# mcmilk/7-Zip-zstd

Hardware: AMD Instinct MI355X
Metric: compress MB/s + ratio-vs-ref, enwik9 zstd-L3 & Silesia flzma2-L5 (value = the zstd-L3 enwik9 leg; flzma2_l5_silesia = the other leg) (higher is better)
Workload: dtype u8; 1 GPU; zstd level 3, enwik9 stand-in (text-zipf, 1000000000 B), 128 KiB blocks in independent 8 MiB match-finder frames; bytes_total=1000000000

## Files before the change

### 7-zip-zstd_amd/csrc/gc_api.hip

```cpp
#include "gpucodec.h"
#include "gc_common.h"
#include "gc_lzma2.h"
#include "gc_brotli.h"
#include "gc_mf.h"
#include "gc_zstd_dec.h"
#include "gc_brotli_dec.h"
#include "gc_lzma2_dec_work.h"
#ifdef HIPEMU
#include "hip_runtime_stub.h"
#else
#include <hip/hip_runtime.h>
#define GC_LAUNCH(kernel, grid, block, stream, ...) hipLaunchKernelGGL(kernel, dim3(grid), dim3(block), 0, stream, __VA_ARGS__)
#endif
#include <stdio.h>
#include <stdlib.h>
#include <string.h>
#include <new>
#include "gc_host_stream.h"
#ifdef GC_TEST_HOOKS
#include <vector>
#include <unistd.h>
#endif

struct GcFramePlan { uint64_t off; uint32_t size; uint32_t compressed; };
// ... 399 lines not shown
#define GC_MF_ENT_BUDGET ((size_t)24u << 30)
static uint32_t mf_auto_parts(size_t n, uint32_t frameArg)
{
    if (MF_F(frameArg) <= 1u) return 1u;
    const size_t perGroup = (size_t)MF_FPG(frameArg) * MF_F(frameArg) * GC_ZSTD_BLOCK_MAX * sizeof(GcMfEntry);
    const size_t nGroups = (gc_num_blocks(n) + MF_C(frameArg) - 1u) / MF_C(frameArg);
    size_t perPart = GC_MF_ENT_BUDGET / perGroup; if (perPart < 1u) perPart = 1u;
    size_t parts = (nGroups + perPart - 1u) / perPart;
    return (uint32_t)(parts < 1u ? 1u : (parts > GC_MAX_PARTS ? GC_MAX_PARTS : parts));
}
static int ensure_finder_workspace(gc_ctx* c, const GcLzPlan& plan, size_t n, uint32_t frameBlocks, size_t maxPartBytes = 0 )
{
    if (MF_F(frameBlocks) <= 1u) return GC_OK;
    const GcMfGeom g = gc_mf_geom(n, frameBlocks, plan.mfFast != 0u);
    const GcMfGeom gp = gc_mf_geom(maxPartBytes && maxPartBytes < n ? maxPartBytes : n, frameBlocks, plan.mfFast != 0u);
    const size_t needCnt = gp.cntWords * sizeof(uint32_t), needEnt = (size_t)gp.nFrames * gp.frameBytes * sizeof(GcMfEntry);
    const size_t needRec = (size_t)g.nBlocks * GC_ZSTD_BLOCK_MAX * sizeof(uint32_t);
    const size_t needPrice = (size_t)g.nBlocks * GC_PRICE_WORDS * sizeof(uint16_t);
    const size_t needTileWord = ((size_t)g.nTiles + 64u) * sizeof(uint32_t);
    if (needTileWord > c->mfTileWordCap || needCnt > c->mfCntCap || needEnt > c->mfEntCap || needEnt > c->mfEnt2Cap || needRec > c->mfRecCap || ((plan.searchDepth || plan.shortPass) && (needRec > c->mfRec2Cap || needRec / 32u + 64u > c->mfChangedCap)) ||
        (plan.priceParse && (needRec / 2u > c->mfRec3Cap || needRec > c->mfDpCap || needPrice > c->mfPriceCap || (size_t)g.nBlocks * 128u > c->mfWinCostCap || (size_t)g.nBlocks * GC_DPS_WORDS * 4u > c->mfDpStatCap || needRec / 4u > c->mfLitPriceCap))) {
        HIPCHK(c, hipStreamSynchronize(c->stream));
        int rc;
        if ((rc = mf_grow(c, (void**)&c->mfTileWord, &c->mfTileWordCap, needTileWord, "tile counts")) != GC_OK) return rc;
        if ((rc = mf_grow(c, (void**)&c->mfCnt, &c->mfCntCap, needCnt, "offsets")) != GC_OK) return rc;
        if ((rc = mf_grow(c, (void**)&c->mfEnt, &c->mfEntCap, needEnt, "entries")) != GC_OK) return rc;
        if ((rc = mf_grow(c, (void**)&c->mfEnt2, &c->mfEnt2Cap, needEnt, "linked entries")) != GC_OK) return rc;
        if ((rc = mf_grow(c, (void**)&c->mfRec, &c->mfRecCap, needRec, "records")) != GC_OK) return rc;
        if ((plan.searchDepth || plan.shortPass) && (rc = mf_grow(c, (void**)&c->mfRec2, &c->mfRec2Cap, needRec, "deepened records")) != GC_OK) return rc;
        if ((plan.searchDepth || plan.shortPass) && (rc = mf_grow(c, (void**)&c->mfChanged, &c->mfChangedCap, needRec / 32u + 64u, "changed-record bitmap")) != GC_OK) return rc;
        if (plan.priceParse) {
            if ((rc = mf_grow(c, (void**)&c->mfRec3, &c->mfRec3Cap, needRec / 2u, "short candidates")) != GC_OK) return rc;
            if ((rc = mf_grow(c, (void**)&c->mfDp, &c->mfDpCap, needRec, "price-parse records")) != GC_OK) return rc;
            if ((rc = mf_grow(c, (void**)&c->mfPrice, &c->mfPriceCap, needPrice, "price tables")) != GC_OK) return rc;
            if ((rc = mf_grow(c, (void**)&c->mfWinCost, &c->mfWinCostCap, (size_t)g.nBlocks * 128u, "window costs")) != GC_OK) return rc;
            if ((rc = mf_grow(c, (void**)&c->mfDpStat, &c->mfDpStatCap, (size_t)g.nBlocks * GC_DPS_WORDS * 4u, "path symbol counts")) != GC_OK) return rc;
            if ((rc = mf_grow(c, (void**)&c->mfLitPrice, &c->mfLitPriceCap, needRec / 4u, "literal prices")) != GC_OK) return rc;
        }
    }
    return GC_OK;
}

static int launch_finder_part(gc_ctx* c, const GcLzPlan& plan, hipStream_t st, uint32_t part, const uint8_t* src, size_t n, uint32_t frameArg , uint32_t blk0, unsigned long long* prof)
{
    const uint32_t frameBlocks = frameArg;
    const uint32_t groupBlocks = MF_C(frameArg);
    const uint32_t nBlocks = gc_num_blocks(n);
    GcSeqRaw* seqRaw = c->seqRaw + (size_t)blk0 * GC_MAX_SEQ_PER_BLOCK;
    uint8_t* lit = c->lit + (size_t)blk0 * GC_ZSTD_BLOCK_MAX;
    GcBlockMeta* meta = c->meta + blk0;
    if (MF_F(frameArg) <= 1u) {
        GC_LAUNCH(gc_zstd_lz_kernel, nBlocks, 1024, st, src, (uint64_t)n, seqRaw, lit, meta, prof);
        return GC_OK;
    }
    const GcMfGeom g = gc_mf_geom(n, frameBlocks, plan.mfFast != 0u);
    const uint32_t frame0 = (blk0 / groupBlocks) * MF_FPG(frameArg);
    uint32_t* cnt = c->mfCnt;
    GcMfEntry* ent = c->mfEnt;
    GcMfEntry* ent2 = c->mfEnt2;
    uint32_t* rec = c->mfRec + (size_t)blk0 * GC_ZSTD_BLOCK_MAX;
    const uint32_t perT = gc_xcd_per(g.nTiles), perB = gc_xcd_per(nBlocks);
    const bool fast = plan.mfFast != 0u;
    const uint32_t nParts = 1u << g.partLog;
#define MFSEL(k) (fast ? k##_p8 : k)
    uint32_t linkLaunch = 0;
    const uint32_t linkWpc = 6u;
    const uint32_t nLists = g.nFrames * nParts, linkGrid = nLists * GC_MF_LINK_SEGS < c->nCU * linkWpc ? nLists * GC_MF_LINK_SEGS : c->nCU * linkWpc;
    HIPCHK(c, hipMemsetAsync(c->mfTicket + part * 16u, 0, 16u * sizeof(uint32_t), st));
#define MF_LINK(cnt_, ent_, ent2_) do { uint32_t* ticket_ = c->mfTicket + part * 16u + linkLaunch++; \
        GC_LAUNCH(MFSEL(gc_mf_link_kernel), linkGrid, 64, st, (const uint32_t*)(cnt_), (const GcMfEntry*)(ent_), ent2_, g.tilesPerFrame, g.frameBytes, nLists, ticket_); } while (0)
    hipEvent_t* ev = c->evMf[part];
    HIPCHK(c, hipEventRecord(ev[0], st));
    const bool shortBeside = plan.priceParse && st == c->stream;
    if (shortBeside) {
        HIPCHK(c, hipEventRecord(c->evShort[part], st)); HIPCHK(c, hipStreamWaitEvent(c->stream2, c->evShort[part], 0));
        const uint32_t nChunkWg = (uint32_t)(((n + 2047u) / 2048u + 3u) / 4u), perC = gc_xcd_per(nChunkWg);
        GC_LAUNCH(gc_mf_short_kernel, perC * GC_XCDS, 256, c->stream2, src, (uint64_t)n, groupBlocks, (uint32_t)((n + 2047u) / 2048u), perC, c->mfRec3 + (size_t)blk0 * GC_ZSTD_BLOCK_MAX);
        HIPCHK(c, hipEventRecord(c->evShort[part], c->stream2));
    }
    GC_LAUNCH(MFSEL(gc_mf_count_kernel), perT * GC_XCDS, nParts, st, src, (uint64_t)n, frameBlocks, g.nTiles, perT, cnt);
    HIPCHK(c, hipEventRecord(ev[1], st));
    GC_LAUNCH(MFSEL(gc_mf_scan_kernel), g.nFrames, 1024, st, cnt, g.tilesPerFrame);
    HIPCHK(c, hipEventRecord(ev[2], st));
    GC_LAUNCH(MFSEL(gc_mf_scatter_kernel), perT * GC_XCDS, nParts, st, src, (uint64_t)n, frameBlocks, g.nTiles, perT, (const uint32_t*)cnt, ent);
    HIPCHK(c, hipEventRecord(ev[3], st));
    MF_LINK(cnt, ent, ent2);
    HIPCHK(c, hipEventRecord(ev[4], st));
    const bool fused = !plan.farPass && !plan.farPass2 && !plan.searchDepth && !plan.priceParse && !plan.shortPass && MF_C(frameArg) == MF_F(frameArg);
    if (fused) {
        {
            const uint32_t tpb = GC_ZSTD_BLOCK_MAX >> g.tileLog;
            const uint32_t perV = ((gc_xcd_per(g.nTiles) + tpb - 1u) / tpb) * tpb;
            uint32_t* tw = c->mfTileWord + (size_t)frame0 * g.tilesPerFrame;
            HIPCHK(c, hipMemsetAsync(tw, 0, (size_t)g.nTiles * sizeof(uint32_t), st));
            GC_LAUNCH(MFSEL(gc_mf_vparse_tile_kernel), perV * GC_XCDS, g.verifyT, st, src, (uint64_t)n, frameBlocks, g.nTiles, perV, plan.lazyDepth, (const uint32_t*)cnt,
                      (const GcMfEntry*)ent2, seqRaw, lit, meta, c->mfTicket + part * 16u + 8u, tw, prof);
        }
        for (int i = 10; i <= 12; i++) HIPCHK(c, hipEventRecord(ev[i], st));
        HIPCHK(c, hipEventRecord(ev[5], st));
        HIPCHK(c, hipEventRecord(ev[6], st));
        (void)prof;
        return GC_OK;
    }
    GC_LAUNCH(MFSEL(gc_mf_verify_kernel), perT * GC_XCDS, g.verifyT, st, src, (uint64_t)n, frameBlocks, g.nTiles, perT, (const uint32_t*)cnt,
                   (const GcMfEntry*)ent2, rec);
    HIPCHK(c, hipEventRecord(ev[10], st));
    if (plan.farPass) {
        GC_LAUNCH(MFSEL(gc_mf_count_far_kernel), perT * GC_XCDS, nParts, st, src, (uint64_t)n, frameBlocks, g.nTiles, perT, cnt);
        GC_LAUNCH(MFSEL(gc_mf_scan_kernel), g.nFrames, 1024, st, cnt, g.tilesPerFrame);
        GC_LAUNCH(MFSEL(gc_mf_scatter_far_kernel), perT * GC_XCDS, nParts, st, src, (uint64_t)n, frameBlocks, g.nTiles, perT, (const uint32_t*)cnt, ent);
        MF_LINK(cnt, ent, ent2);
        GC_LAUNCH(MFSEL(gc_mf_verify_far_kernel), perT * GC_XCDS, g.verifyT, st, src, (uint64_t)n, frameBlocks, g.nTiles, perT, (const uint32_t*)cnt,
                  (const GcMfEntry*)ent2, rec);
    }
    if (plan.farPass2) {
        GC_LAUNCH(MFSEL(gc_mf_count_far2_kernel), perT * GC_XCDS, nParts, st, src, (uint64_t)n, frameBlocks, g.nTiles, perT, cnt);
        GC_LAUNCH(MFSEL(gc_mf_scan_kernel), g.nFrames, 1024, st, cnt, g.tilesPerFrame);
        GC_LAUNCH(MFSEL(gc_mf_scatter_far2_kernel), perT * GC_XCDS, nParts, st, src, (uint64_t)n, frameBlocks, g.nTiles, perT, (const uint32_t*)cnt, ent);
        MF_LINK(cnt, ent, ent2);
        GC_LAUNCH(MFSEL(gc_mf_verify_far2_kernel), perT * GC_XCDS, g.verifyT, st, src, (uint64_t)n, frameBlocks, g.nTiles, perT, (const uint32_t*)cnt,
                  (const GcMfEntry*)ent2, rec);
    }
    HIPCHK(c, hipEventRecord(ev[11], st));
    uint32_t* const chg = (plan.searchDepth && plan.shortPass && plan.priceParse) ? c->mfChanged + (size_t)blk0 * (GC_ZSTD_BLOCK_MAX / 32u) : (uint32_t*)nullptr;
    if (plan.searchDepth) {
        uint32_t* rec2 = c->mfRec2 + (size_t)blk0 * GC_ZSTD_BLOCK_MAX;
        GC_LAUNCH(MFSEL(gc_mf_deepen_kernel), perT * GC_XCDS, 256, st, src, (uint64_t)n, frameBlocks, g.nTiles, perT, plan.searchDepth | (plan.searchShallow << 8), (const uint32_t*)rec, rec2, chg);
        rec = rec2;
    }
    HIPCHK(c, hipEventRecord(ev[12], st));
    const uint32_t litCtxArg = plan.priceLitCtx | (blk0 != 0u ? 0x80000000u : 0u);
    const uint32_t* recDp = rec;
    if (plan.priceParse && plan.shortPass) {
        uint32_t* recN = rec == c->mfRec + (size_t)blk0 * GC_ZSTD_BLOCK_MAX ? c->mfRec2 + (size_t)blk0 * GC_ZSTD_BLOCK_MAX : c->mfRec + (size_t)blk0 * GC_ZSTD_BLOCK_MAX;
        const uint32_t fbS = plan.shortPlain ? MF_F(frameArg) : frameArg;
        const GcMfGeom gs = gc_mf_geom(n, fbS, plan.mfFast != 0u);
        const uint32_t perTs = gc_xcd_per(gs.nTiles), nListsS = gs.nFrames * nParts;
        uint32_t* cntS = c->mfCnt;
        GC_LAUNCH(MFSEL(gc_mf_count_short_kernel), perTs * GC_XCDS, nParts, st, src, (uint64_t)n, fbS, gs.nTiles, perTs, cntS);
        GC_LAUNCH(MFSEL(gc_mf_scan_kernel), gs.nFrames, 1024, st, cntS, gs.tilesPerFrame);
        GC_LAUNCH(MFSEL(gc_mf_scatter_short_kernel), perTs * GC_XCDS, nParts, st, src, (uint64_t)n, fbS, gs.nTiles, perTs, (const uint32_t*)cntS, ent);
        {   uint32_t* ticket_ = c->mfTicket + part * 16u + linkLaunch++;
            const uint32_t gridS = nListsS * GC_MF_LINK_SEGS < c->nCU * linkWpc ? nListsS * GC_MF_LINK_SEGS : c->nCU * linkWpc;
            GC_LAUNCH(MFSEL(gc_mf_link_kernel), gridS, 64, st, (const uint32_t*)cntS, (const GcMfEntry*)ent, ent2, gs.tilesPerFrame, gs.frameBytes, nListsS, ticket_); }
        if (plan.shortPlain) GC_LAUNCH(MFSEL(gc_mf_verify_short_kernel), perTs * GC_XCDS, gs.verifyT, st, src, (uint64_t)n, fbS, gs.nTiles, perTs, (const uint32_t*)cntS,
                  (const GcMfEntry*)ent2, (const uint32_t*)rec, recN, (const uint32_t*)chg);
        else GC_LAUNCH(MFSEL(gc_mf_verify_shortb_kernel), perTs * GC_XCDS, gs.verifyT, st, src, (uint64_t)n, fbS, gs.nTiles, perTs, (const uint32_t*)cntS,
                  (const GcMfEntry*)ent2, (const uint32_t*)rec, recN, (const uint32_t*)chg);
        recDp = recN;
    }
    HIPCHK(c, hipEventRecord(ev[5], st));
    if (plan.priceParse) {
        uint16_t* price = c->mfPrice + (size_t)blk0 * GC_PRICE_WORDS;
        uint16_t* rec3 = c->mfRec3 + (size_t)blk0 * GC_ZSTD_BLOCK_MAX;
        uint32_t* dp = c->mfDp + (size_t)blk0 * GC_ZSTD_BLOCK_MAX;
        uint32_t* wc = c->mfWinCost + (size_t)blk0 * 32u;
        GC_LAUNCH(gc_mf_parse_kernel, perB * GC_XCDS, GC_MF_PARSE_T, st, src, (uint64_t)n, nBlocks, perB, plan.lazyDepth, (const uint32_t*)rec, seqRaw, lit, meta, price, litCtxArg);
        HIPCHK(c, hipEventRecord(ev[7], st));
        const uint32_t nChunkWg = (uint32_t)(((n + 2047u) / 2048u + 3u) / 4u), perC = gc_xcd_per(nChunkWg);
        if (shortBeside) HIPCHK(c, hipStreamWaitEvent(st, c->evShort[part], 0));
        else GC_LAUNCH(gc_mf_short_kernel, perC * GC_XCDS, 256, st, src, (uint64_t)n, groupBlocks, (uint32_t)((n + 2047u) / 2048u), perC, rec3);
        HIPCHK(c, hipEventRecord(ev[8], st));
        uint32_t* dps = c->mfDpStat + (size_t)blk0 * GC_DPS_WORDS;
        HIPCHK(c, hipMemsetAsync(dps, 0, (size_t)nBlocks * GC_DPS_WORDS * sizeof(uint32_t), st));
        uint8_t* lpr = c->mfLitPrice + (size_t)blk0 * GC_ZSTD_BLOCK_MAX;
        if (plan.laneDp) GC_LAUNCH(gc_mf_litprice_kernel, perB * GC_XCDS, 256, st, src, (uint64_t)n, nBlocks, perB, (const uint16_t*)price, litCtxArg, lpr);
        for (uint32_t pass = plan.dpPhases == 1u ? 1u : 0u; pass < 2u; pass++) {
            const uint32_t phase = plan.dpPhases == 1u ? 2u : pass;
            const uint32_t nDpWg = nBlocks * (phase == 0u ? 1u : 8u), perD = gc_xcd_per(nDpWg);
            uint32_t* wcp = phase == 0u ? (uint32_t*)nullptr : wc;
            if (plan.laneDp) {
                const bool w2 = (plan.smallWin2k == 2u || (plan.smallWin2k == 1u && nBlocks <= 1024u)) && phase != 0u;
                const uint32_t nItems = w2 ? nBlocks : (nBlocks + 1u) / 2u, perL = gc_xcd_per(nItems);
                const bool select = plan.laneDp == 2u && phase == 1u && !w2;
                const uint32_t phaseK = phase | (w2 ? 16u : 0u) | (select ? GC_DP_SELECT : 0u) | (plan.allLengths ? GC_DP_ALLLEN : 0u);
                if (select) {
                    if (plan.priceMinLen <= 2u) GC_LAUNCH(gc_mf_dp2_kernel, perD * GC_XCDS, 256, st, src, (uint64_t)n, nBlocks, perD, groupBlocks, phaseK, dps, litCtxArg, recDp, (const uint16_t*)rec3, (const uint16_t*)price, dp, wcp);
                    else GC_LAUNCH(gc_mf_dp3_kernel, perD * GC_XCDS, 256, st, src, (uint64_t)n, nBlocks, perD, groupBlocks, phaseK, dps, litCtxArg, recDp, (const uint16_t*)rec3, (const uint16_t*)price, dp, wcp);
                }
                if (plan.priceMinLen <= 2u) {
                    if (phase == 0u) GC_LAUNCH(gc_mf_dpl2s_kernel, perL * GC_XCDS, GC_DPL_THREADS, st, src, (uint64_t)n, nBlocks, perL, groupBlocks, phase | (plan.allLengths ? GC_DP_ALLLEN : 0u), dps, litCtxArg, recDp, (const uint16_t*)rec3, (const uint16_t*)price, dp, wcp, (const uint8_t*)lpr);
                    else GC_LAUNCH(gc_mf_dpl2_kernel, perL * GC_XCDS, GC_DPL_THREADS, st, src, (uint64_t)n, nBlocks, perL, groupBlocks, phaseK, dps, litCtxArg, recDp, (const uint16_t*)rec3, (const uint16_t*)price, dp, wcp, (const uint8_t*)lpr);
                } else {
                    if (phase == 0u) GC_LAUNCH(gc_mf_dplzs_kernel, perL * GC_XCDS, GC_DPL_THREADS, st, src, (uint64_t)n, nBlocks, perL, groupBlocks, phase | (plan.allLengths ? GC_DP_ALLLEN : 0u), dps, litCtxArg, recDp, (const uint16_t*)rec3, (const uint16_t*)price, dp, wcp, (const uint8_t*)lpr);
                    else GC_LAUNCH(gc_mf_dplz_kernel, perL * GC_XCDS, GC_DPL_THREADS, st, src, (uint64_t)n, nBlocks, perL, groupBlocks, phaseK, dps, litCtxArg, recDp, (const uint16_t*)rec3, (const uint16_t*)price, dp, wcp, (const uint8_t*)lpr);
                }
            } else
            if (plan.priceMinLen <= 2u) GC_LAUNCH(gc_mf_dp2_kernel, perD * GC_XCDS, 256, st, src, (uint64_t)n, nBlocks, perD, groupBlocks, phase, dps, litCtxArg, recDp, (const uint16_t*)rec3, (const uint16_t*)price, dp, wcp);
            else GC_LAUNCH(gc_mf_dp3_kernel, perD * GC_XCDS, 256, st, src, (uint64_t)n, nBlocks, perD, groupBlocks, phase, dps, litCtxArg, recDp, (const uint16_t*)rec3, (const uint16_t*)price, dp, wcp);
        }
        HIPCHK(c, hipEventRecord(ev[9], st));
        GC_LAUNCH(gc_mf_parse_kernel, perB * GC_XCDS, GC_MF_PARSE_T, st, src, (uint64_t)n, nBlocks, perB, 0u, (const uint32_t*)dp, seqRaw, lit, meta, (uint16_t*)nullptr, 0u);
    } else if (plan.ringParse) {
        if ((plan.ringParse >> 8) & 0xFFu)
            GC_LAUNCH(gc_mf_parse_kernel, perB * GC_XCDS, GC_MF_PARSE_T, st, src, (uint64_t)n, nBlocks, perB, plan.lazyDepth, (const uint32_t*)rec, seqRaw, lit, meta, (uint16_t*)nullptr, 0u);
        GC_LAUNCH(gc_mf_ringparse_kernel, perB * GC_XCDS, plan.ringGeom, st, src, (uint64_t)n, nBlocks, perB, plan.lazyDepth < 1u ? plan.lazyDepth : 1u, plan.ringParse, (const uint32_t*)rec, seqRaw, lit, meta);
    }
    else
        GC_LAUNCH(gc_mf_parse_kernel, perB * GC_XCDS, GC_MF_PARSE_T, st, src, (uint64_t)n, nBlocks, perB, plan.lazyDepth, (const uint32_t*)rec, seqRaw, lit, meta, (uint16_t*)nullptr, 0u);
    HIPCHK(c, hipEventRecord(ev[6], st));
    (void)prof;
    return GC_OK;
}

static int launch_finder(gc_ctx* c, const GcLzPlan& plan, const uint8_t* src, size_t n, uint32_t frameBlocks, unsigned long long* prof)
{
    c->mfTimed = false;
    int rc = ensure_finder_workspace(c, plan, n, frameBlocks);
    if (rc != GC_OK) return rc;
    rc = launch_finder_part(c, plan, c->stream, 0, src, n, frameBlocks, 0, prof);
    if (rc != GC_OK) return rc;
    c->mfTimed = MF_F(frameBlocks) > 1u; c->mfParts = 1; c->mfPriced = c->mfTimed && plan.priceParse != 0u;
    return GC_OK;
}

extern "C" int gc_mf_last_timing(gc_ctx* c, float ms[6])
{
    if (!c || !c->timed || c->pending || !c->mfTimed) return GC_ERR_PARAM;
    for (int i = 0; i < 6; i++) ms[i] = 0.f;
    for (uint32_t p = 0; p < c->mfParts; p++)
        for (int i = 0; i < 6; i++) { float t = 0.f; HIPCHK(c, hipEventElapsedTime(&t, c->evMf[p][i], c->evMf[p][i + 1])); ms[i] += t; }
    return GC_OK;
}

// ... 874 lines not shown
```

### 7-zip-zstd_amd/csrc/gc_lz_window.hip

```cpp
#include "gc_mf.h"
#include "gc_lz_parse.h"
#ifdef HIPEMU
#include <stdio.h>
#include <stdlib.h>
#endif

#ifdef GC_MF_FAST
#define MFK(name) name##_p8
#else
#define MFK(name) name
#endif

namespace MFK(gc_mf_ns) {

#define MF_T         GC_MF_PARTS
#define MF_WAVES     (MF_T / 64u)
static_assert(MF_T == GC_MF_PARTS, "W1/W3 use one thread per partition for the histogram rows");
#define MF_STAGE_PAD 16u
#define MF_STAGE_WORDS ((GC_MF_TILE + 2u * MF_STAGE_PAD + 32u) / 4u)

__device__ __forceinline__ uint32_t mf_item(uint32_t bid, uint32_t per) { return (bid & (GC_XCDS - 1u)) * per + (bid >> 3); }

struct MfTile {
    uint32_t frame, tif;
    uint64_t frameStart, frameEnd;
    uint64_t tileStart;
    uint32_t len;
    bool own;
};
__device__ __forceinline__ MfTile mf_tile(uint32_t tile, uint32_t frameBlocks, uint64_t srcSize)
{
    MfTile T;
    const uint32_t F = MF_F(frameBlocks), S = MF_S(frameBlocks), C = MF_C(frameBlocks), fpg = 1u + (C - F) / S;
    const uint32_t TPF = F * GC_MF_TILES_PER_BLOCK;
    const uint64_t frameBytes = (uint64_t)F * GC_ZSTD_BLOCK_MAX;
    T.frame = tile / TPF; T.tif = tile % TPF;
    const uint32_t gi = T.frame / fpg, fi = T.frame % fpg;
    const uint64_t groupStart = (uint64_t)gi * C * GC_ZSTD_BLOCK_MAX;
    const uint64_t groupEnd = (groupStart + (uint64_t)C * GC_ZSTD_BLOCK_MAX) < srcSize ? (groupStart + (uint64_t)C * GC_ZSTD_BLOCK_MAX) : srcSize;
    T.frameStart = groupStart + (uint64_t)fi * S * GC_ZSTD_BLOCK_MAX;
    T.frameEnd = (T.frameStart + frameBytes) < groupEnd ? (T.frameStart + frameBytes) : groupEnd;
    T.tileStart = T.frameStart + (uint64_t)T.tif * GC_MF_TILE;
    T.len = T.tileStart < T.frameEnd ? (uint32_t)((T.frameEnd - T.tileStart) < GC_MF_TILE ? (T.frameEnd - T.tileStart) : GC_MF_TILE) : 0u;
    T.own = fi == 0u || T.tif >= (F - S) * GC_MF_TILES_PER_BLOCK;
    return T;
}

__device__ __forceinline__ void mf_stage(uint32_t* sW, uint32_t nWords, const uint8_t* __restrict__ src, uint64_t srcSize, uint64_t tileStart, uint32_t t, uint32_t nThreads)
{
    for (uint32_t c = t; c < nWords / 4u; c += nThreads) {
        GcU4 v; v.x = v.y = v.z = v.w = 0;
        if (tileStart + 16ull * c >= MF_STAGE_PAD) {
            const uint64_t pos = tileStart + 16ull * c - MF_STAGE_PAD;
            if (pos + 16u <= srcSize) __builtin_memcpy(&v, src + pos, 16);
            else if (pos < srcSize) { uint8_t tmp[16]; for (uint32_t i = 0; i < 16u; i++) tmp[i] = pos + i < srcSize ? src[pos + i] : (uint8_t)0; __builtin_memcpy(&v, tmp, 16); }
        }
        sW[4u * c] = v.x; sW[4u * c + 1u] = v.y; sW[4u * c + 2u] = v.z; sW[4u * c + 3u] = v.w;
    }
}
__device__ __forceinline__ uint64_t mf_lds_ld64(const uint32_t* sW, uint32_t i)
{
    const uint32_t w = i >> 2, sh = (i & 3u) * 8u;
    const uint32_t w0 = sW[w], w1 = sW[w + 1u], w2 = sW[w + 2u];
    const uint32_t lo = (uint32_t)((((uint64_t)w1 << 32) | w0) >> sh);
    const uint32_t hi = (uint32_t)((((uint64_t)w2 << 32) | w1) >> sh);
    return ((uint64_t)hi << 32) | lo;
}
__device__ __forceinline__ uint32_t mf_lds_byte(const uint32_t* sW, uint32_t i) { return (sW[i >> 2] >> ((i & 3u) * 8u)) & 0xFFu; }

#define MF_BASE  0
#define MF_FAR   1
#define MF_SHORT 2
#define MF_FAR2  4
struct MfKeys { bool ok, run; uint32_t part; uint64_t entry; };
template <int MODE>
__device__ __forceinline__ MfKeys mf_keys(const uint32_t* sW, uint32_t q, const MfTile& T)
{
    MfKeys r; r.ok = false; r.run = false; r.part = 0; r.entry = 0;
    const uint64_t P = T.tileStart + q;
    const uint64_t x = mf_lds_ld64(sW, q + MF_STAGE_PAD);
    if (P > T.frameStart) r.run = ((x << 8) | (uint64_t)mf_lds_byte(sW, q + MF_STAGE_PAD - 1u)) == x;
    if (q < T.len && P + GC_MATCH_CAP + 16u <= T.frameEnd && !r.run) {
        const uint32_t lo = (uint32_t)x, hi = (uint32_t)(x >> 32);
        uint32_t hL = lz_hash_long(lo, hi), hS = lz_hash_short(lo, hi);
        if (MODE == MF_SHORT) {
            if (((lo ^ (lo >> 8)) & 0xFFFFu) == 0u) return r;
            hS = (lo & 0xFFFFFFu) * 0x9E3779B1u; hS ^= hS >> 15; hS *= 0x2C1B3C6Du;
            hL = lo * 0x9E3779B1u; hL ^= hL >> 15; hL *= 0x85EBCA77u;
        }
        if (MODE == MF_FAR2) {
            const uint64_t y = mf_lds_ld64(sW, q + MF_STAGE_PAD + 8u), z = mf_lds_ld64(sW, q + MF_STAGE_PAD + 16u), w = mf_lds_ld64(sW, q + MF_STAGE_PAD + 24u);
            uint32_t h = hL + (uint32_t)y * 0xC2B2AE3Du; h ^= h >> 15; h *= 0x2C1B3C6Du;
            h += (uint32_t)(y >> 32) * 0x27D4EB2Fu; h ^= h >> 13; h *= 0x165667B1u;
            h += (uint32_t)z * 0x9E3779B1u; h ^= h >> 16; h *= 0x85EBCA6Bu;
            hS = h + (uint32_t)(z >> 32) * 0xC2B2AE35u;
            hS ^= hS >> 15; hS *= 0x2C1B3C6Du;
            hL = hS + (uint32_t)w * 0x27D4EB2Fu; hL ^= hL >> 13; hL *= 0x165667B1u;
            hL += (uint32_t)(w >> 32) * 0x9E3779B1u;
            hL ^= hL >> 16; hL *= 0x85EBCA77u;
        }
// ... 18 lines not shown
__device__ __forceinline__ void mf_count_body(const uint8_t* __restrict__ src, uint64_t srcSize, uint32_t frameBlocks, uint32_t nTiles, uint32_t per, uint32_t* __restrict__ cnt)
{
    __shared__ uint32_t sW[MF_STAGE_WORDS];
    __shared__ uint32_t sHist[GC_MF_PARTS];
    const uint32_t t = threadIdx.x;
    const uint32_t tile = mf_item(blockIdx.x, per);
    if (tile >= nTiles) return;
    const MfTile T = mf_tile(tile, frameBlocks, srcSize);
    const uint32_t TPF = MF_F(frameBlocks) * GC_MF_TILES_PER_BLOCK;
    sHist[t] = 0;
    if (T.len) mf_stage(sW, MF_STAGE_WORDS, src, srcSize, T.tileStart, t, MF_T);
    __syncthreads();
    for (uint32_t q = t; q < T.len; q += MF_T) {
        const MfKeys k = mf_keys<MODE>(sW, q, T);
        if (k.ok) atomicAdd(&sHist[k.part], 1u);
    }
    __syncthreads();
    cnt[((uint64_t)T.frame * (TPF + 1u) + T.tif) * GC_MF_PARTS + t] = sHist[t];
}
extern "C" __global__ void __launch_bounds__(MF_T)
MFK(gc_mf_count_kernel)(const uint8_t* __restrict__ src, uint64_t srcSize, uint32_t frameBlocks, uint32_t nTiles, uint32_t per, uint32_t* __restrict__ cnt)
{
    mf_count_body<MF_BASE>(src, srcSize, frameBlocks, nTiles, per, cnt);
}
extern "C" __global__ void __launch_bounds__(MF_T)
MFK(gc_mf_count_short_kernel)(const uint8_t* __restrict__ src, uint64_t srcSize, uint32_t frameBlocks, uint32_t nTiles, uint32_t per, uint32_t* __restrict__ cnt)
{
    mf_count_body<MF_SHORT>(src, srcSize, frameBlocks, nTiles, per, cnt);
}
extern "C" __global__ void __launch_bounds__(MF_T)
MFK(gc_mf_count_far_kernel)(const uint8_t* __restrict__ src, uint64_t srcSize, uint32_t frameBlocks, uint32_t nTiles, uint32_t per, uint32_t* __restrict__ cnt)
{
    mf_count_body<MF_FAR>(src, srcSize, frameBlocks, nTiles, per, cnt);
}
extern "C" __global__ void __launch_bounds__(MF_T)
MFK(gc_mf_count_far2_kernel)(const uint8_t* __restrict__ src, uint64_t srcSize, uint32_t frameBlocks, uint32_t nTiles, uint32_t per, uint32_t* __restrict__ cnt)
{
    mf_count_body<MF_FAR2>(src, srcSize, frameBlocks, nTiles, per, cnt);
}

extern "C" __global__ void __launch_bounds__(1024)
MFK(gc_mf_scan_kernel)(uint32_t* __restrict__ cnt, uint32_t tilesPerFrame)
{
    constexpr uint32_t Q = 1024u / GC_MF_PARTS;
    constexpr uint32_t NW = GC_MF_PARTS / 64u;
    __shared__ uint32_t sPart[Q][GC_MF_PARTS];
    __shared__ uint32_t sStart[GC_MF_PARTS];
    __shared__ uint32_t sWave[NW];
    const uint32_t t = threadIdx.x, lane = t & 63u, wave = t >> 6, q = t >> GC_MF_PART_LOG, g = t & (GC_MF_PARTS - 1u);
    uint32_t* A = cnt + (uint64_t)blockIdx.x * (tilesPerFrame + 1u) * GC_MF_PARTS;
    const uint32_t R = (tilesPerFrame + Q - 1u) / Q;
    const uint32_t r0 = q * R < tilesPerFrame ? q * R : tilesPerFrame, r1 = (q + 1u) * R < tilesPerFrame ? (q + 1u) * R : tilesPerFrame;
    uint32_t sum = 0;
    for (uint32_t r = r0; r < r1; r++) sum += A[(uint64_t)r * GC_MF_PARTS + g];
    sPart[q][g] = sum;
    __syncthreads();
    uint32_t tot = 0, incl = 0;
    if (t < GC_MF_PARTS) {
        for (uint32_t qq = 0; qq < Q; qq++) tot += sPart[qq][t];
        incl = gc_wave_incl_sum(tot);
        if (lane == 63u) sWave[wave] = incl;
    }
    __syncthreads();
    if (t < GC_MF_PARTS) {
        uint32_t before = 0;
        for (uint32_t w = 0; w < NW; w++) if (w < wave) before += sWave[w];
        sStart[t] = before + incl - tot;
    }
    __syncthreads();
    uint32_t run = sStart[g];
    for (uint32_t qq = 0; qq < Q; qq++) if (qq < q) run += sPart[qq][g];
    for (uint32_t r = r0; r < r1; r++) {
        const uint64_t i = (uint64_t)r * GC_MF_PARTS + g;
        const uint32_t v = A[i]; A[i] = run; run += v;
    }
    if (q == Q - 1u) A[(uint64_t)tilesPerFrame * GC_MF_PARTS + g] = run;
}

template <int MODE>
__device__ __forceinline__ void mf_scatter_body(const uint8_t* __restrict__ src, uint64_t srcSize, uint32_t frameBlocks, uint32_t nTiles, uint32_t per,
                     const uint32_t* __restrict__ offs, GcMfEntry* __restrict__ ent)
{
    __shared__ uint32_t sW[MF_STAGE_WORDS];
    __shared__ uint32_t sRun[MF_WAVES][GC_MF_PARTS];
    __shared__ uint32_t sLocal[GC_MF_PARTS], sGlob[GC_MF_PARTS];
    __shared__ uint32_t sWaveTot[MF_WAVES];
    __shared__ uint16_t sPerm[GC_MF_TILE];
    const uint32_t t = threadIdx.x, lane = t & 63u, wave = t >> 6;
    const uint32_t tile = mf_item(blockIdx.x, per);
    if (tile >= nTiles) return;
    const MfTile T = mf_tile(tile, frameBlocks, srcSize);
    if (T.len == 0u) return;
    const uint32_t TPF = MF_F(frameBlocks) * GC_MF_TILES_PER_BLOCK;
    for (uint32_t w = 0; w < MF_WAVES; w++) sRun[w][t] = 0;
    mf_stage(sW, MF_STAGE_WORDS, src, srcSize, T.tileStart, t, MF_T);
    __syncthreads();
    const uint32_t qBase = wave * (GC_MF_TILE / MF_WAVES);
    for (uint32_t r = 0; r < GC_MF_TILE / MF_T; r++) {
        const MfKeys k = mf_keys<MODE>(sW, qBase + r * 64u + lane, T);
        if (k.ok) atomicAdd(&sRun[wave][k.part], 1u);
    }
    __syncthreads();
    uint32_t c[MF_WAVES], tot = 0;
    for (uint32_t w = 0; w < MF_WAVES; w++) { c[w] = sRun[w][t]; tot += c[w]; }
    const uint32_t incl = gc_wave_incl_sum(tot);
    if (lane == 63u) sWaveTot[wave] = incl;
    __syncthreads();
    {
        uint32_t before = 0;
        for (uint32_t w = 0; w < MF_WAVES; w++) if (w < wave) before += sWaveTot[w];
        uint32_t ls = before + incl - tot;
        sLocal[t] = ls;
        for (uint32_t w = 0; w < MF_WAVES; w++) { sRun[w][t] = ls; ls += c[w]; }
        sGlob[t] = offs[((uint64_t)T.frame * (TPF + 1u) + T.tif) * GC_MF_PARTS + t];
    }
    __syncthreads();
    uint32_t nEnt = 0;
    for (uint32_t w = 0; w < MF_WAVES; w++) nEnt += sWaveTot[w];
    for (uint32_t r = 0; r < GC_MF_TILE / MF_T; r++) {
        const uint32_t q = qBase + r * 64u + lane;
        const MfKeys k = mf_keys<MODE>(sW, q, T);
        if (k.ok) sPerm[atomicAdd(&sRun[wave][k.part], 1u)] = (uint16_t)q;
        gc_wave_step();
    }
    __syncthreads();
    GcMfEntry* E = ent + (uint64_t)T.frame * ((uint64_t)MF_F(frameBlocks) * GC_ZSTD_BLOCK_MAX);
    for (uint32_t j = t; j < nEnt; j += MF_T) {
        const MfKeys k = mf_keys<MODE>(sW, sPerm[j], T);
        E[sGlob[k.part] + (j - sLocal[k.part])] = k.entry;
    }
}
extern "C" __global__ void __launch_bounds__(MF_T)
MFK(gc_mf_scatter_kernel)(const uint8_t* __restrict__ src, uint64_t srcSize, uint32_t frameBlocks, uint32_t nTiles, uint32_t per,
                     const uint32_t* __restrict__ offs, GcMfEntry* __restrict__ ent)
{
    mf_scatter_body<MF_BASE>(src, srcSize, frameBlocks, nTiles, per, offs, ent);
}
extern "C" __global__ void __launch_bounds__(MF_T)
MFK(gc_mf_scatter_short_kernel)(const uint8_t* __restrict__ src, uint64_t srcSize, uint32_t frameBlocks, uint32_t nTiles, uint32_t per,
                           const uint32_t* __restrict__ offs, GcMfEntry* __restrict__ ent)
{
    mf_scatter_body<MF_SHORT>(src, srcSize, frameBlocks, nTiles, per, offs, ent);
}
extern "C" __global__ void __launch_bounds__(MF_T)
MFK(gc_mf_scatter_far_kernel)(const uint8_t* __restrict__ src, uint64_t srcSize, uint32_t frameBlocks, uint32_t nTiles, uint32_t per,
                         const uint32_t* __restrict__ offs, GcMfEntry* __restrict__ ent)
{
    mf_scatter_body<MF_FAR>(src, srcSize, frameBlocks, nTiles, per, offs, ent);
}
extern "C" __global__ void __launch_bounds__(MF_T)
MFK(gc_mf_scatter_far2_kernel)(const uint8_t* __restrict__ src, uint64_t srcSize, uint32_t frameBlocks, uint32_t nTiles, uint32_t per,
                         const uint32_t* __restrict__ offs, GcMfEntry* __restrict__ ent)
{
    mf_scatter_body<MF_FAR2>(src, srcSize, frameBlocks, nTiles, per, offs, ent);
}

#ifndef LINK_DEPTH
#define LINK_DEPTH 8u
#endif
#ifdef GC_MF_FAST
#define LINK_SEG   49152u
#else
#define LINK_SEG   16384u
#endif
#define LINK_WARM  16384u
#define LINK_SEGS  GC_MF_LINK_SEGS
#define LINK_BATCH 16u

__device__ __forceinline__ uint32_t mf_link_pick(uint32_t seen, uint32_t mine)
{
    return (seen != 0u && seen < mine && ((seen ^ mine) & ((1u << GC_MF_TAG_BITS) - 1u)) == 0u) ? (seen >> GC_MF_TAG_BITS) : 0u;
}

__device__ __forceinline__ void mf_link_load(uint64_t q[LINK_DEPTH], const GcMfEntry* __restrict__ E, uint32_t s0, uint32_t end, uint32_t lane)
{
#pragma unroll
    for (uint32_t d = 0; d < LINK_DEPTH; d++) {
        const uint32_t i = s0 + d * 64u + lane;
        q[d] = E[i < end ? i : end - 1u];
    }
}

__device__ __forceinline__ void mf_link_steps(const uint64_t q[LINK_DEPTH], uint32_t* tabL, uint32_t* tabS, GcMfEntry* __restrict__ EO, uint32_t s0,
                                              uint32_t end, uint32_t lane)
{
    if (s0 >= end) return;
    uint32_t pos[LINK_DEPTH], mL[LINK_DEPTH], mS[LINK_DEPTH], rL[LINK_DEPTH], rS[LINK_DEPTH];
#pragma unroll
    for (uint32_t d = 0; d < LINK_DEPTH; d++) {
        const uint32_t i = s0 + d * 64u + lane;
        const uint64_t e = q[d];
        pos[d] = (uint32_t)e & ((1u << GC_MF_POS_BITS) - 1u);
        const uint32_t kL = (uint32_t)(e >> GC_MF_POS_BITS) & ((1u << GC_MF_KL_BITS) - 1u);
        const uint32_t kS = (uint32_t)(e >> (GC_MF_POS_BITS + GC_MF_KL_BITS)) & ((1u << GC_MF_KS_BITS) - 1u);
        mL[d] = ((pos[d] + 1u) << GC_MF_TAG_BITS) | (kL & ((1u << GC_MF_TAG_BITS) - 1u)); mS[d] = ((pos[d] + 1u) << GC_MF_TAG_BITS) | (kS & ((1u << GC_MF_TAG_BITS) - 1u));
        rL[d] = 0; rS[d] = 0;
        if (i < end) { rL[d] = atomicMax(&tabL[kL >> (GC_MF_KL_BITS - GC_MF_LSLOT_LOG)], mL[d]); rS[d] = atomicMax(&tabS[kS >> (GC_MF_KS_BITS - GC_MF_SSLOT_LOG)], mS[d]); }
        gc_wave_step();
    }
#pragma unroll
    for (uint32_t d = 0; d < LINK_DEPTH; d++) {
        const uint32_t i = s0 + d * 64u + lane;
        const uint32_t cL = mf_link_pick(rL[d], mL[d]), cS = mf_link_pick(rS[d], mS[d]);
        if (i < end) EO[i] = (uint64_t)(pos[d] & (GC_MF_TILE - 1u)) | ((uint64_t)cL << GC_MF_TILE_LOG) | ((uint64_t)cS << (GC_MF_TILE_LOG + GC_MF_CAND_BITS));
    }
}

extern "C" __global__ void __launch_bounds__(64)
MFK(gc_mf_link_kernel)(const uint32_t* __restrict__ offs, const GcMfEntry* __restrict__ ent, GcMfEntry* __restrict__ entOut, uint32_t tilesPerFrame,
                  uint64_t frameBytes, uint32_t nLists, uint32_t* __restrict__ ticket)
{
    __shared__ uint32_t tabL[1u << GC_MF_LSLOT_LOG];
    __shared__ uint32_t tabS[1u << GC_MF_SSLOT_LOG];
    const uint32_t lane = threadIdx.x;
    const uint32_t nUpper = nLists * (LINK_SEGS - 1u), nBatches = (nUpper + LINK_BATCH - 1u) / LINK_BATCH, nTickets = nBatches + nLists;
    for (;;) {
        uint32_t tk = 0;
        if (lane == 0u) tk = atomicAdd(ticket, 1u);
        tk = __shfl(tk, 0);
        if (tk >= nTickets) break;
        uint64_t todo;
        uint32_t myItem, myStart = 0, myEnd = 0;
        {
            myItem = tk < nBatches ? tk * LINK_BATCH + lane : nUpper + (tk - nBatches);
            const bool inRange = tk < nBatches ? (lane < LINK_BATCH && myItem < nUpper) : lane == 0u;
            bool exists = false;
            if (inRange) {
                const uint32_t seg = LINK_SEGS - 1u - myItem / nLists, fg = myItem % nLists;
                const uint32_t frame = fg >> GC_MF_PART_LOG, g = fg & (GC_MF_PARTS - 1u);
                const uint32_t* row = offs + (uint64_t)frame * (tilesPerFrame + 1u) * GC_MF_PARTS;
                const uint32_t listStart = row[g], listEnd = row[(uint64_t)tilesPerFrame * GC_MF_PARTS + g];
                myStart = listStart + seg * LINK_SEG;
                exists = myStart < listEnd;
// ... 921 lines not shown
```

### 7-zip-zstd_amd/csrc/gc_mf.h

```cpp
#pragma once
#include <stdint.h>
#include "gc_common.h"

#define GC_MF_WIDE_TILE_LOG 14u
#define GC_MF_WIDE_PART_LOG 10u
#define GC_MF_WIDE_VERIFY_T 1024u
#define GC_MF_FAST_TILE_LOG 13u
#define GC_MF_FAST_PART_LOG 8u
#define GC_MF_FAST_VERIFY_T 512u
#ifdef GC_MF_FAST
#define GC_MF_TILE_LOG    GC_MF_FAST_TILE_LOG
#define GC_MF_PART_LOG    GC_MF_FAST_PART_LOG
#else
#define GC_MF_TILE_LOG    GC_MF_WIDE_TILE_LOG
#define GC_MF_PART_LOG    GC_MF_WIDE_PART_LOG
#endif
#define GC_MF_TILE        (1u << GC_MF_TILE_LOG)
#define GC_MF_TILES_PER_BLOCK (GC_ZSTD_BLOCK_MAX >> GC_MF_TILE_LOG)
#define GC_MF_PARTS       (1u << GC_MF_PART_LOG)
#define GC_MF_MAX_FRAME_BLOCKS 64u
#define GC_MF_WIDE_MAX_FRAME_BLOCKS 128u

typedef uint64_t GcMfEntry;
#ifdef GC_MF_FAST
#define GC_MF_POS_BITS    23u
#define GC_MF_TAG_BITS    8u
#else
#define GC_MF_POS_BITS    24u
#define GC_MF_TAG_BITS    7u
#endif
#define GC_MF_CAND_BITS   (GC_MF_POS_BITS + 1u)
#define GC_MF_KL_BITS     20u
#define GC_MF_KS_BITS     19u
#ifndef GC_MF_LSLOT_LOG
#define GC_MF_LSLOT_LOG   12u
#endif
#ifndef GC_MF_SSLOT_LOG
#define GC_MF_SSLOT_LOG   11u
#endif

#define GC_MF_PARSE_T     1024u
#ifdef GC_MF_FAST
#define GC_MF_VERIFY_T    GC_MF_FAST_VERIFY_T
#else
#define GC_MF_VERIFY_T    GC_MF_WIDE_VERIFY_T
#endif
#define GC_MF_LINK_SEGS   8u

#define GC_MF_GEOM_ARG(F, S, C) ((uint32_t)(F) | ((uint32_t)(S) << 8) | ((uint32_t)(C) << 16))
#define MF_F(a) ((a) & 0xFFu)
#define MF_S(a) ((((a) >> 8) & 0xFFu) ? (((a) >> 8) & 0xFFu) : MF_F(a))
#define MF_C(a) (((a) >> 16) ? ((a) >> 16) : MF_F(a))
#define MF_FPG(a) (1u + (MF_C(a) - MF_F(a)) / MF_S(a))

struct GcMfGeom {
    uint32_t tileLog, partLog, verifyT;
    uint32_t frameBlocks;
    uint32_t nBlocks;
    uint32_t nFrames;
    uint32_t tilesPerFrame;
    uint32_t nTiles;
    uint64_t frameBytes;
    uint64_t cntWords;
};

static inline GcMfGeom gc_mf_geom(uint64_t n, uint32_t frameArg, bool fast)
{
    GcMfGeom g;
    const uint32_t frameBlocks = MF_F(frameArg);
    g.tileLog = fast ? GC_MF_FAST_TILE_LOG : GC_MF_WIDE_TILE_LOG; g.partLog = fast ? GC_MF_FAST_PART_LOG : GC_MF_WIDE_PART_LOG;
    g.verifyT = fast ? GC_MF_FAST_VERIFY_T : GC_MF_WIDE_VERIFY_T;
    g.frameBlocks = frameBlocks;
    g.nBlocks = gc_num_blocks(n);
    g.nFrames = ((g.nBlocks + MF_C(frameArg) - 1u) / MF_C(frameArg)) * MF_FPG(frameArg);
    g.tilesPerFrame = frameBlocks * (GC_ZSTD_BLOCK_MAX >> g.tileLog);
    g.nTiles = g.nFrames * g.tilesPerFrame;
    g.frameBytes = (uint64_t)frameBlocks * GC_ZSTD_BLOCK_MAX;
    g.cntWords = (uint64_t)g.nFrames * (g.tilesPerFrame + 1u) << g.partLog;
    return g;
}

#define GC_PRICE_LIT    0u
#define GC_PRICE_LEN    2048u
#define GC_PRICE_NLEN   80u
#define GC_PRICE_SLOT   (GC_PRICE_LEN + GC_PRICE_NLEN)
#define GC_PRICE_FLAGS  (GC_PRICE_SLOT + 64u)
#define GC_PRICE_REPLEN (GC_PRICE_FLAGS + 8u)
#define GC_PRICE_WORDS  (GC_PRICE_REPLEN + GC_PRICE_NLEN)
#define GC_PRICE_MAX    240u
#define GC_DPS_LEN      0u
#define GC_DPS_SLOT     GC_PRICE_NLEN
#define GC_DPS_NLIT     (GC_DPS_SLOT + 64u)
#define GC_DPS_NMAT     (GC_DPS_NLIT + 1u)
#define GC_DPS_NREP      (GC_DPS_NLIT + 2u)
#define GC_DPS_NSREP     (GC_DPS_NLIT + 3u)
#define GC_DPS_NREP1     (GC_DPS_NLIT + 4u)
#define GC_DPS_NREP2     (GC_DPS_NLIT + 5u)
#define GC_DPS_NREP3     (GC_DPS_NLIT + 6u)
#define GC_DPS_REPLEN   160u
#define GC_DPS_WORDS    240u
#ifndef GC_DPL_THREADS
#define GC_DPL_THREADS  128u
#endif
#define GC_DP_SELECT    32u
#define GC_DP_ALLLEN    128u
#define GC_DPS_RICH(C)  ((C)[GC_DPS_NMAT] != 0u && ((C)[GC_DPS_NREP] + (C)[GC_DPS_NSREP] + (C)[GC_DPS_NREP1] + (C)[GC_DPS_NREP2] + (C)[GC_DPS_NREP3]) * 20u >= (C)[GC_DPS_NMAT])
#define GC_SHORT_NONE   0xFFFFu

#define GC_XCDS 8u
static inline uint32_t gc_xcd_per(uint32_t n) { return (n + GC_XCDS - 1u) / GC_XCDS; }
```

Baseline: 44990 MB/s.

## Decouple match-finder scatter block size from partition count and cache keys

The scatter kernels now launch with a dedicated thread count (1024 wide / 512 fast) instead of one thread per partition. Only the first GC_MF_PARTS threads compute the per-partition offsets, and the two global/local offset arrays become a single delta array. Each thread packs the partition IDs from the histogram pass into registers, so the permutation pass no longer recomputes the hash keys. The aim is more parallelism per tile and less redundant key work, paid for with more registers and more per-wave sRun rows in shared memory, which may reduce occupancy.

```diff
diff --git a/7-zip-zstd_amd/csrc/gc_api.hip b/7-zip-zstd_amd/csrc/gc_api.hip
--- a/7-zip-zstd_amd/csrc/gc_api.hip
+++ b/7-zip-zstd_amd/csrc/gc_api.hip
@@ -505,7 +505,7 @@
     HIPCHK(c, hipEventRecord(ev[1], st));
     GC_LAUNCH(MFSEL(gc_mf_scan_kernel), g.nFrames, 1024, st, cnt, g.tilesPerFrame);
     HIPCHK(c, hipEventRecord(ev[2], st));
-    GC_LAUNCH(MFSEL(gc_mf_scatter_kernel), perT * GC_XCDS, nParts, st, src, (uint64_t)n, frameBlocks, g.nTiles, perT, (const uint32_t*)cnt, ent);
+    GC_LAUNCH(MFSEL(gc_mf_scatter_kernel), perT * GC_XCDS, g.scatterT, st, src, (uint64_t)n, frameBlocks, g.nTiles, perT, (const uint32_t*)cnt, ent);
     HIPCHK(c, hipEventRecord(ev[3], st));
     MF_LINK(cnt, ent, ent2);
     HIPCHK(c, hipEventRecord(ev[4], st));
@@ -531,7 +531,7 @@
     if (plan.farPass) {
         GC_LAUNCH(MFSEL(gc_mf_count_far_kernel), perT * GC_XCDS, nParts, st, src, (uint64_t)n, frameBlocks, g.nTiles, perT, cnt);
         GC_LAUNCH(MFSEL(gc_mf_scan_kernel), g.nFrames, 1024, st, cnt, g.tilesPerFrame);
-        GC_LAUNCH(MFSEL(gc_mf_scatter_far_kernel), perT * GC_XCDS, nParts, st, src, (uint64_t)n, frameBlocks, g.nTiles, perT, (const uint32_t*)cnt, ent);
+        GC_LAUNCH(MFSEL(gc_mf_scatter_far_kernel), perT * GC_XCDS, g.scatterT, st, src, (uint64_t)n, frameBlocks, g.nTiles, perT, (const uint32_t*)cnt, ent);
         MF_LINK(cnt, ent, ent2);
         GC_LAUNCH(MFSEL(gc_mf_verify_far_kernel), perT * GC_XCDS, g.verifyT, st, src, (uint64_t)n, frameBlocks, g.nTiles, perT, (const uint32_t*)cnt,
                   (const GcMfEntry*)ent2, rec);
@@ -539,7 +539,7 @@
     if (plan.farPass2) {
         GC_LAUNCH(MFSEL(gc_mf_count_far2_kernel), perT * GC_XCDS, nParts, st, src, (uint64_t)n, frameBlocks, g.nTiles, perT, cnt);
         GC_LAUNCH(MFSEL(gc_mf_scan_kernel), g.nFrames, 1024, st, cnt, g.tilesPerFrame);
-        GC_LAUNCH(MFSEL(gc_mf_scatter_far2_kernel), perT * GC_XCDS, nParts, st, src, (uint64_t)n, frameBlocks, g.nTiles, perT, (const uint32_t*)cnt, ent);
+        GC_LAUNCH(MFSEL(gc_mf_scatter_far2_kernel), perT * GC_XCDS, g.scatterT, st, src, (uint64_t)n, frameBlocks, g.nTiles, perT, (const uint32_t*)cnt, ent);
         MF_LINK(cnt, ent, ent2);
         GC_LAUNCH(MFSEL(gc_mf_verify_far2_kernel), perT * GC_XCDS, g.verifyT, st, src, (uint64_t)n, frameBlocks, g.nTiles, perT, (const uint32_t*)cnt,
                   (const GcMfEntry*)ent2, rec);
@@ -562,7 +562,7 @@
         uint32_t* cntS = c->mfCnt;
         GC_LAUNCH(MFSEL(gc_mf_count_short_kernel), perTs * GC_XCDS, nParts, st, src, (uint64_t)n, fbS, gs.nTiles, perTs, cntS);
         GC_LAUNCH(MFSEL(gc_mf_scan_kernel), gs.nFrames, 1024, st, cntS, gs.tilesPerFrame);
-        GC_LAUNCH(MFSEL(gc_mf_scatter_short_kernel), perTs * GC_XCDS, nParts, st, src, (uint64_t)n, fbS, gs.nTiles, perTs, (const uint32_t*)cntS, ent);
+        GC_LAUNCH(MFSEL(gc_mf_scatter_short_kernel), perTs * GC_XCDS, gs.scatterT, st, src, (uint64_t)n, fbS, gs.nTiles, perTs, (const uint32_t*)cntS, ent);
         {   uint32_t* ticket_ = c->mfTicket + part * 16u + linkLaunch++;
             const uint32_t gridS = nListsS * GC_MF_LINK_SEGS < c->nCU * linkWpc ? nListsS * GC_MF_LINK_SEGS : c->nCU * linkWpc;
             GC_LAUNCH(MFSEL(gc_mf_link_kernel), gridS, 64, st, (const uint32_t*)cntS, (const GcMfEntry*)ent, ent2, gs.tilesPerFrame, gs.frameBytes, nListsS, ticket_); }
diff --git a/7-zip-zstd_amd/csrc/gc_lz_window.hip b/7-zip-zstd_amd/csrc/gc_lz_window.hip
--- a/7-zip-zstd_amd/csrc/gc_lz_window.hip
+++ b/7-zip-zstd_amd/csrc/gc_lz_window.hip
@@ -14,8 +14,12 @@
 namespace MFK(gc_mf_ns) {
 
 #define MF_T         GC_MF_PARTS
-#define MF_WAVES     (MF_T / 64u)
-static_assert(MF_T == GC_MF_PARTS, "W1/W3 use one thread per partition for the histogram rows");
+static_assert(MF_T == GC_MF_PARTS, "W1 uses one thread per partition for the histogram row");
+#define MF_PWAVES    (GC_MF_PARTS / 64u)
+#define MFS_T        GC_MF_SCATTER_T
+#define MFS_WAVES    (MFS_T / 64u)
+#define MFS_ROUNDS   (GC_MF_TILE / MFS_T)
+static_assert(MFS_T >= GC_MF_PARTS && MFS_T % 64u == 0u && GC_MF_TILE % (2u * MFS_T) == 0u && GC_MF_PARTS < 0xFFFFu, "W3: the first GC_MF_PARTS threads do the offsets; whole rounds, two per register");
 #define MF_STAGE_PAD 16u
 #define MF_STAGE_WORDS ((GC_MF_TILE + 2u * MF_STAGE_PAD + 32u) / 4u)
 
@@ -200,9 +204,9 @@
                      const uint32_t* __restrict__ offs, GcMfEntry* __restrict__ ent)
 {
     __shared__ uint32_t sW[MF_STAGE_WORDS];
-    __shared__ uint32_t sRun[MF_WAVES][GC_MF_PARTS];
-    __shared__ uint32_t sLocal[GC_MF_PARTS], sGlob[GC_MF_PARTS];
-    __shared__ uint32_t sWaveTot[MF_WAVES];
+    __shared__ uint32_t sRun[MFS_WAVES][GC_MF_PARTS];
+    __shared__ uint32_t sDelta[GC_MF_PARTS];
+    __shared__ uint32_t sWaveTot[MF_PWAVES];
     __shared__ uint16_t sPerm[GC_MF_TILE];
     const uint32_t t = threadIdx.x, lane = t & 63u, wave = t >> 6;
     const uint32_t tile = mf_item(blockIdx.x, per);
@@ -210,63 +214,68 @@
     const MfTile T = mf_tile(tile, frameBlocks, srcSize);
     if (T.len == 0u) return;
     const uint32_t TPF = MF_F(frameBlocks) * GC_MF_TILES_PER_BLOCK;
-    for (uint32_t w = 0; w < MF_WAVES; w++) sRun[w][t] = 0;
-    mf_stage(sW, MF_STAGE_WORDS, src, srcSize, T.tileStart, t, MF_T);
-    __syncthreads();
-    const uint32_t qBase = wave * (GC_MF_TILE / MF_WAVES);
-    for (uint32_t r = 0; r < GC_MF_TILE / MF_T; r++) {
+    for (uint32_t i = t; i < MFS_WAVES * GC_MF_PARTS; i += MFS_T) (&sRun[0][0])[i] = 0;
+    mf_stage(sW, MF_STAGE_WORDS, src, srcSize, T.tileStart, t, MFS_T);
+    __syncthreads();
+    const uint32_t qBase = wave * (GC_MF_TILE / MFS_WAVES);
+    uint32_t pk[MFS_ROUNDS / 2u];
+#pragma unroll
+    for (uint32_t r = 0; r < MFS_ROUNDS; r++) {
         const MfKeys k = mf_keys<MODE>(sW, qBase + r * 64u + lane, T);
+        const uint32_t p = k.ok ? k.part : 0xFFFFu;
+        pk[r >> 1] = (r & 1u) ? (pk[r >> 1] | (p << 16)) : p;
         if (k.ok) atomicAdd(&sRun[wave][k.part], 1u);
     }
     __syncthreads();
-    uint32_t c[MF_WAVES], tot = 0;
-    for (uint32_t w = 0; w < MF_WAVES; w++) { c[w] = sRun[w][t]; tot += c[w]; }
-    const uint32_t incl = gc_wave_incl_sum(tot);
-    if (lane == 63u) sWaveTot[wave] = incl;
-    __syncthreads();
-    {
+    uint32_t tot = 0, incl = 0;
+    if (t < GC_MF_PARTS) {
+        for (uint32_t w = 0; w < MFS_WAVES; w++) tot += sRun[w][t];
+        incl = gc_wave_incl_sum(tot);
+        if (lane == 63u) sWaveTot[wave] = incl;
+    }
+    __syncthreads();
+    if (t < GC_MF_PARTS) {
         uint32_t before = 0;
-        for (uint32_t w = 0; w < MF_WAVES; w++) if (w < wave) before += sWaveTot[w];
+        for (uint32_t w = 0; w < MF_PWAVES; w++) if (w < wave) before += sWaveTot[w];
         uint32_t ls = before + incl - tot;
-        sLocal[t] = ls;
-        for (uint32_t w = 0; w < MF_WAVES; w++) { sRun[w][t] = ls; ls += c[w]; }
-        sGlob[t] = offs[((uint64_t)T.frame * (TPF + 1u) + T.tif) * GC_MF_PARTS + t];
+        sDelta[t] = offs[((uint64_t)T.frame * (TPF + 1u) + T.tif) * GC_MF_PARTS + t] - ls;
+        for (uint32_t w = 0; w < MFS_WAVES; w++) { const uint32_t c = sRun[w][t]; sRun[w][t] = ls; ls += c; }
     }
     __syncthreads();
     uint32_t nEnt = 0;
-    for (uint32_t w = 0; w < MF_WAVES; w++) nEnt += sWaveTot[w];
-    for (uint32_t r = 0; r < GC_MF_TILE / MF_T; r++) {
-        const uint32_t q = qBase + r * 64u + lane;
-        const MfKeys k = mf_keys<MODE>(sW, q, T);
-        if (k.ok) sPerm[atomicAdd(&sRun[wave][k.part], 1u)] = (uint16_t)q;
+    for (uint32_t w = 0; w < MF_PWAVES; w++) nEnt += sWaveTot[w];
+#pragma unroll
+    for (uint32_t r = 0; r < MFS_ROUNDS; r++) {
+        const uint32_t p = (pk[r >> 1] >> ((r & 1u) * 16u)) & 0xFFFFu;
+        if (p != 0xFFFFu) sPerm[atomicAdd(&sRun[wave][p], 1u)] = (uint16_t)(qBase + r * 64u + lane);
         gc_wave_step();
     }
     __syncthreads();
     GcMfEntry* E = ent + (uint64_t)T.frame * ((uint64_t)MF_F(frameBlocks) * GC_ZSTD_BLOCK_MAX);
-    for (uint32_t j = t; j < nEnt; j += MF_T) {
+    for (uint32_t j = t; j < nEnt; j += MFS_T) {
         const MfKeys k = mf_keys<MODE>(sW, sPerm[j], T);
-        E[sGlob[k.part] + (j - sLocal[k.part])] = k.entry;
-    }
-}
-extern "C" __global__ void __launch_bounds__(MF_T)
+        E[sDelta[k.part] + j] = k.entry;
+    }
+}
+extern "C" __global__ void __launch_bounds__(MFS_T)
 MFK(gc_mf_scatter_kernel)(const uint8_t* __restrict__ src, uint64_t srcSize, uint32_t frameBlocks, uint32_t nTiles, uint32_t per,
                      const uint32_t* __restrict__ offs, GcMfEntry* __restrict__ ent)
 {
     mf_scatter_body<MF_BASE>(src, srcSize, frameBlocks, nTiles, per, offs, ent);
 }
-extern "C" __global__ void __launch_bounds__(MF_T)
+extern "C" __global__ void __launch_bounds__(MFS_T)
 MFK(gc_mf_scatter_short_kernel)(const uint8_t* __restrict__ src, uint64_t srcSize, uint32_t frameBlocks, uint32_t nTiles, uint32_t per,
                            const uint32_t* __restrict__ offs, GcMfEntry* __restrict__ ent)
 {
     mf_scatter_body<MF_SHORT>(src, srcSize, frameBlocks, nTiles, per, offs, ent);
 }
-extern "C" __global__ void __launch_bounds__(MF_T)
+extern "C" __global__ void __launch_bounds__(MFS_T)
 MFK(gc_mf_scatter_far_kernel)(const uint8_t* __restrict__ src, uint64_t srcSize, uint32_t frameBlocks, uint32_t nTiles, uint32_t per,
                          const uint32_t* __restrict__ offs, GcMfEntry* __restrict__ ent)
 {
     mf_scatter_body<MF_FAR>(src, srcSize, frameBlocks, nTiles, per, offs, ent);
 }
-extern "C" __global__ void __launch_bounds__(MF_T)
+extern "C" __global__ void __launch_bounds__(MFS_T)
 MFK(gc_mf_scatter_far2_kernel)(const uint8_t* __restrict__ src, uint64_t srcSize, uint32_t frameBlocks, uint32_t nTiles, uint32_t per,
                          const uint32_t* __restrict__ offs, GcMfEntry* __restrict__ ent)
 {
diff --git a/7-zip-zstd_amd/csrc/gc_mf.h b/7-zip-zstd_amd/csrc/gc_mf.h
--- a/7-zip-zstd_amd/csrc/gc_mf.h
+++ b/7-zip-zstd_amd/csrc/gc_mf.h
@@ -8,6 +8,8 @@
 #define GC_MF_FAST_TILE_LOG 13u
 #define GC_MF_FAST_PART_LOG 8u
 #define GC_MF_FAST_VERIFY_T 512u
+#define GC_MF_WIDE_SCATTER_T 1024u
+#define GC_MF_FAST_SCATTER_T 512u
 #ifdef GC_MF_FAST
 #define GC_MF_TILE_LOG    GC_MF_FAST_TILE_LOG
 #define GC_MF_PART_LOG    GC_MF_FAST_PART_LOG
@@ -42,7 +44,9 @@
 #define GC_MF_PARSE_T     1024u
 #ifdef GC_MF_FAST
 #define GC_MF_VERIFY_T    GC_MF_FAST_VERIFY_T
+#define GC_MF_SCATTER_T   GC_MF_FAST_SCATTER_T
 #else
+#define GC_MF_SCATTER_T   GC_MF_WIDE_SCATTER_T
 #define GC_MF_VERIFY_T    GC_MF_WIDE_VERIFY_T
 #endif
 #define GC_MF_LINK_SEGS   8u
@@ -54,7 +58,7 @@
 #define MF_FPG(a) (1u + (MF_C(a) - MF_F(a)) / MF_S(a))
 
 struct GcMfGeom {
-    uint32_t tileLog, partLog, verifyT;
+    uint32_t tileLog, partLog, verifyT, scatterT;
     uint32_t frameBlocks;
     uint32_t nBlocks;
     uint32_t nFrames;
@@ -69,7 +73,7 @@
     GcMfGeom g;
     const uint32_t frameBlocks = MF_F(frameArg);
     g.tileLog = fast ? GC_MF_FAST_TILE_LOG : GC_MF_WIDE_TILE_LOG; g.partLog = fast ? GC_MF_FAST_PART_LOG : GC_MF_WIDE_PART_LOG;
-    g.verifyT = fast ? GC_MF_FAST_VERIFY_T : GC_MF_WIDE_VERIFY_T;
+    g.verifyT = fast ? GC_MF_FAST_VERIFY_T : GC_MF_WIDE_VERIFY_T; g.scatterT = fast ? GC_MF_FAST_SCATTER_T : GC_MF_WIDE_SCATTER_T;
     g.frameBlocks = frameBlocks;
     g.nBlocks = gc_num_blocks(n);
     g.nFrames = ((g.nBlocks + MF_C(frameArg) - 1u) / MF_C(frameArg)) * MF_FPG(frameArg);
```

After: 46200 MB/s (median of 6 runs). +2.7%, better.
